# chenhaoxing/DiffUTE

Measured on AMD Instinct MI355X. Metric: 512x512 50-step denoise images/sec, higher is better.
Workload: dtype bf16; 1 GPU; SD2-inpaint UNet 50-step DDIM denoise loop, 512x512 px, batch 4 per GPU, glyph context [B,577,1024], ctx K/V cached per image (BASELINE configs[1]); VAE encode/decode not in the timed region; global_batch=4, denoise_steps=50, parallelism=replicas x1 (no collective), weights=random-init SD2-inpainting shapes (865,925,124 params), bf16 packed

## Files before the change

### diffute_amd/csrc/exec.h

```cpp
#pragma once
#include <map>
#include <string>
#include <unordered_map>
#include <vector>
#include "kernels.h"

struct PackRule {
  enum Kind { COPY_F32, CONV, LINEAR, GEGLU_W, GEGLU_B } kind = COPY_F32;
  size_t dst = 0;
  int rows = 0, cols = 0;
  int ks = 0, ld = 0, koff = 0;
};
struct ParamEntry { std::string name; int shape[4]; PackRule rule; };

class ParamTable {
 public:
  size_t reserve(size_t bytes) { size_t o = total_; total_ += align_up(bytes, 256); return o; }
  void add(const std::string& name, std::initializer_list<int> shape, const PackRule& r) {
    ParamEntry e; e.name = name; int i = 0; for (int k = 0; k < 4; ++k) e.shape[k] = 0;
    for (int s : shape) e.shape[i++] = s;
    e.rule = r; index_[name] = (int)entries_.size(); entries_.push_back(e);
  }
  size_t f32(const std::string& name, int n) {
    PackRule r; r.kind = PackRule::COPY_F32; r.dst = reserve((size_t)n * 4); r.rows = n; add(name, {n}, r); return r.dst;
// ... 85 lines not shown

struct ConvOpts {
  int ksize = 3, stride = 1, pad = 1, ups = 0;
  const float* bias2 = nullptr;
  int ldw = 0;
  int ups2 = 0;
  const float* bias = nullptr;
  const float* rowbias = nullptr; int ldrb = 0;
  const Tn* res = nullptr;
  const Tn* sc0 = nullptr; const Tn* sc1 = nullptr;
  int out_f32 = 0;
  int stats = 0;
  int defer = 0;
};

class Exec {
 public:
  hipStream_t stream = nullptr;
  bool dry = false;
  int rc = 0;
  Workspace ws;
  bool f32 = false;
  bool ff_fold = dmx_ff_fold_enabled();
  const char* masters = nullptr;
  struct Weights {
    const char* base; size_t mul;
    template <typename T> const T* at(size_t off) const { return (const T*)(base + off * mul); }
  };
  Weights weights(const char* arena) const { return f32 ? Weights{masters, 2} : Weights{arena, 1}; }
  static Exec dry_run(bool f32 = false) { Exec e; e.dry = true; e.f32 = f32; e.ws.reset(nullptr, 0, true); return e; }
  static Exec on(hipStream_t stream, void* ws, size_t bytes, bool f32 = false) { Exec e; e.stream = stream; e.f32 = f32; e.ws.reset(ws, bytes, false); return e; }
  TapSink* taps = nullptr;
  size_t esz() const { return f32 ? 4 : 2; }
  bf16* col(const Tn& t, int c) const { return (bf16*)((char*)t.p + (size_t)c * esz()); }
  void tap(const Tn& t);

  Tn make(int B, int H, int W, int C) {
    Tn t; t.B = B; t.H = H; t.W = W; t.C = C; t.ld = C;
    t.p = (bf16*)ws.alloc((size_t)B * H * W * C * esz());
    if (ws.failed() && !rc) { dmx_set_error("workspace too small"); rc = DMX_ERR_WORKSPACE; }
    return t;
  }
  void* raw(size_t bytes) {
    void* p = ws.alloc(bytes);
    if (ws.failed() && !rc) { dmx_set_error("workspace too small"); rc = DMX_ERR_WORKSPACE; }
    return p;
// ... 54 lines not shown
```

### diffute_amd/csrc/exec.hip

```cpp
#include <stdarg.h>
#include <stdio.h>
#include <string.h>
#include "exec.h"
#include <vector>

static thread_local char g_err[512] = "";
void dmx_set_error(const char* fmt, ...) {
  va_list ap; va_start(ap, fmt); vsnprintf(g_err, sizeof(g_err), fmt, ap); va_end(ap);
}
const char* dmx_get_error() { return g_err; }
static int* g_dev_err = nullptr;
int* dmx_dev_err_words() {
  static bool tried = false;
  if (!tried) {
    tried = true;
    void* p = nullptr;
    if (hipHostMalloc(&p, 64, hipHostMallocMapped | hipHostMallocCoherent) == hipSuccess && p) { memset(p, 0, 64); g_dev_err = (int*)p; }
    else (void)hipGetLastError();
  }
  return g_dev_err;
}
int dmx_poll_device_error() {
  volatile int* e = g_dev_err;
  if (!e || !e[0]) return DMX_OK;
// ... 10 lines not shown
  else if (k == DMX_DEVK_ATTN_PEER)
    dmx_set_error("device error: attention (balanced schedule) slot %d gave up after 40 ms waiting for the partial (O, m, l) record of slot %d for query block %d (%d slots) - "
                  "the slots in front of it did not run; the result of that launch is invalid", blk, d0, d1, d2);
  else
    dmx_set_error("device error %d raised by block %d (%d, %d, %d)", k, blk, d0, d1, d2);
  e[0] = 0;
  for (int i = 2; i < 8; ++i) e[i] = 0;
  __atomic_thread_fence(__ATOMIC_SEQ_CST);
  e[1] = 0;
  return DMX_ERR_DEVICE;
}
extern "C" int dmx_device_error(void) { return dmx_poll_device_error(); }
int dmx_check_launch(const char* what) {
  hipError_t e = hipGetLastError();
  if (e != hipSuccess) { dmx_set_error("launch of %s failed: %s", what, hipGetErrorString(e)); return DMX_ERR_HIP; }
  const int rc = dmx_poll_device_error();
  if (rc) {
    char first[400]; strncpy(first, dmx_get_error(), sizeof(first) - 1); first[sizeof(first) - 1] = 0;
    dmx_set_error("%s [surfaced at the launch check of %s, which itself was enqueued correctly; the walk it belongs to is abandoned]", first, what ? what : "?");
  }
  return rc;
}

static int g_plan_sw[DMX_SW_COUNT] = {1, 1, 1, 1, 1, 1, 1, 0, 1, 1, 1, 1};
void dmx_plan_switch(int slot, int value) { if (slot >= 0 && slot < DMX_SW_COUNT) g_plan_sw[slot] = value; }
void dmx_plan_epoch_bump() { ++g_plan_sw[DMX_SW_OVERRIDES]; }
extern "C" int dmx_plan_epoch(void) {
  unsigned h = 2166136261u;
  for (int i = 0; i < DMX_SW_COUNT; ++i) h = (h ^ (unsigned)g_plan_sw[i]) * 16777619u;
  return (int)(h & 0x7fffffffu);
}

namespace {
struct ProfRec { hipEvent_t a, b; int cls; double flops, bytes; char tag[96]; char sym[112]; };
struct ProfSym { char sym[112]; int cls; double n, ms, flops, bytes; };
std::vector<ProfSym> g_prof_syms;
bool g_prof_on = false;
std::vector<ProfRec> g_prof;
char g_prof_path[512] = "";
}
ProfScope::ProfScope(ProfClass c, hipStream_t s, double flops, double bytes, const char* tag) {
  if (!g_prof_on) return;
  ProfRec r; r.cls = c; r.flops = flops; r.bytes = bytes; r.tag[0] = 0; r.sym[0] = 0;
  if (tag) { strncpy(r.tag, tag, sizeof(r.tag) - 1); r.tag[sizeof(r.tag) - 1] = 0; }
  if (hipEventCreate(&r.a) != hipSuccess || hipEventCreate(&r.b) != hipSuccess) return;
  (void)hipEventRecord(r.a, s);
  slot = (int)g_prof.size(); g_prof.push_back(r);
// ... 98 lines not shown
  auto nxt = free_.lower_bound(o);
  if (nxt != free_.end() && o + sz == nxt->first) { sz += nxt->second; nxt = free_.erase(nxt); }
  if (nxt != free_.begin()) {
    auto prv = std::prev(nxt);
    if (prv->first + prv->second == o) { o = prv->first; sz += prv->second; free_.erase(prv); }
  }
  free_[o] = sz;
}

static int g_gn_producer_stats = 1;
extern "C" int dmx_set_gn_producer_stats(int on) { const int old = g_gn_producer_stats; g_gn_producer_stats = on; dmx_plan_switch(DMX_SW_GN_STATS, on); return old; }

static int g_defer_reduce = 1;
extern "C" int dmx_set_defer_reduce(int on) { const int old = g_defer_reduce; g_defer_reduce = on; dmx_plan_switch(DMX_SW_DEFER, on); return old; }

static int g_halo_conv = 1;
extern "C" int dmx_set_halo_conv(int on) { const int old = g_halo_conv; g_halo_conv = on; dmx_plan_switch(DMX_SW_HALO, on); return old; }
bool dmx_halo_conv_enabled() { return g_halo_conv != 0; }

static int g_ff_fold = 1;
extern "C" int dmx_set_ff_fold(int on) { const int old = g_ff_fold; g_ff_fold = on ? 1 : 0; dmx_plan_switch(DMX_SW_FF_FOLD, g_ff_fold); return old; }
bool dmx_ff_fold_enabled() { return g_ff_fold != 0; }

#ifdef DMX_PROBES
static int g_pool_memset_nodes = 0;
static unsigned long long* g_pool_counts = nullptr;
extern "C" int dmx_set_pool_memset_nodes(int mode) { const int old = g_pool_memset_nodes; g_pool_memset_nodes = mode; return old; }
__global__ __launch_bounds__(256) void dmx_probe_count_nonzero_kernel(const u32x4* p, size_t n16, unsigned long long* dst) {
  unsigned long long c = 0;
  for (size_t i = (size_t)blockIdx.x * blockDim.x + threadIdx.x; i < n16; i += (size_t)gridDim.x * blockDim.x) { const u32x4 v = p[i]; c += (v.x | v.y | v.z | v.w) != 0u; }
  if (c) atomicAdd(dst, c);
  if (blockIdx.x == 0 && threadIdx.x == 0 && p[n16 - 1].x != 0u) { dst[4] = p[n16 - 1].x | ((unsigned long long)p[n16 - 1].y << 32); dst[5] = p[n16 / 2].x | ((unsigned long long)p[n16 / 2].y << 32); }
}
extern "C" int dmx_probe_pool_counts(unsigned long long* host8, int reset) {
  if (!g_pool_counts) { DMX_HIP(hipMalloc(&g_pool_counts, 128)); DMX_HIP(hipMemset(g_pool_counts, 0, 128)); }
  DMX_HIP(hipDeviceSynchronize());
  if (host8) DMX_HIP(hipMemcpy(host8, g_pool_counts, 64, hipMemcpyDeviceToHost));
  if (reset) DMX_HIP(hipMemset(g_pool_counts, 0, 128));
  return DMX_OK;
}
#endif
bool Exec::zero_pool(void* p, size_t bytes, int which) {
  if (dry || rc) return !rc;
#ifdef DMX_PROBES
  if (g_pool_memset_nodes & 1) {
    const bool count = (g_pool_memset_nodes & 2) && g_pool_counts;
// ... 93 lines not shown
  Tn y = make(x0.B, x0.H, x0.W, C);
  if (f32) {
    if (!dry && !rc)
      rc = dmx_groupnorm_f32_launch((const float*)x0.p, x0.ld, x0.C, x1 ? (const float*)x1->p : nullptr, x1 ? x1->ld : 0, C, groups, x0.B, x0.H * x0.W,
                                    gamma, beta, eps, silu ? 1 : 0, (float*)y.p, y.ld, stream);
    return y;
  }
  if (x1) flush(*x1);
  if (x0.cst && (!x1 || x1->cst)) {
    flush(x0);
    if (!dry && !rc) {
      GroupNormArgs a{};
      a.x0 = x0.p; a.ldx0 = x0.ld; a.c0 = x0.C;
      a.x1 = x1 ? x1->p : nullptr; a.ldx1 = x1 ? x1->ld : 0;
      a.C = C; a.groups = groups; a.B = x0.B; a.HW = x0.H * x0.W;
      a.gamma = gamma; a.beta = beta; a.eps = eps; a.silu = silu ? 1 : 0;
      a.y = y.p; a.ldy = y.ld; a.st0 = x0.cst; a.st1 = x1 ? x1->cst : x0.cst;
      char tag[96]; snprintf(tag, sizeof(tag), "rows=%d C=%d sums", x0.rows(), C);
      ProfScope ps(PROF_GNORM, stream, 0.0, 4.0 * (double)x0.rows() * C, tag);
      rc = dmx_groupnorm_sums_launch(a, stream);
    }
    return y;
  }
  const size_t pb = dmx_gn_workspace_bytes(x0.B, x0.H * x0.W, groups);
  void* part = raw(pb);
  PendRed* P = (x0.pend >= 0 && x0.pend < (int)pend_.size() && !pend_[x0.pend].done) ? &pend_[x0.pend] : nullptr;
  GroupNormArgs a{};
  a.x0 = x0.p; a.ldx0 = x0.ld; a.c0 = x0.C;
  a.x1 = x1 ? x1->p : nullptr; a.ldx1 = x1 ? x1->ld : 0;
  a.C = C; a.groups = groups; a.B = x0.B; a.HW = x0.H * x0.W;
  a.gamma = gamma; a.beta = beta; a.eps = eps; a.silu = silu ? 1 : 0;
  a.y = y.p; a.ldy = y.ld; a.partial = (float*)part;
  if (P) {
    a.red_partial = P->a.partial ? P->a.partial : (const float*)8;
    a.red_splitk = P->a.splitk; a.red_mn = (long long)P->a.M * P->a.N;
    a.red_bias = P->a.bias; a.red_rowbias = P->a.rowbias; a.red_ldrb = P->a.ldrb; a.red_rpg = P->a.rows_per_group;
    a.red_res = P->a.res; a.red_ldres = P->a.ldres;
    if (P->a.N != x0.C || P->a.ldo != x0.ld || !dmx_gn_red_ok(a)) {
      flush(x0); P = nullptr;
      a.red_partial = nullptr; a.red_splitk = 0;
    }
  }
  if (!dry && !rc) {
    const bool one = dmx_gn_single_launch(a);
    char tag[96]; snprintf(tag, sizeof(tag), "rows=%d C=%d%s%s", x0.rows(), C, one ? " slab" : "", P ? " + split-K reduce" : "");
    ProfScope ps(PROF_GNORM, stream, 0.0, (one ? 4.0 : 6.0) * (double)x0.rows() * C, tag);
    if (!rc) rc = dmx_groupnorm_launch(a, stream);
  }
  if (P) { if (P->wsp) ws.release(P->wsp); P->wsp = nullptr; P->done = true; }
  ws.release(part);
  return y;
}

Tn Exec::conv(const Tn& x0, const Tn* x1, const bf16* w, int Cout, const ConvOpts& o, void* f32_out) {
  flush(x0); if (x1) flush(*x1); if (o.sc0) flush(*o.sc0); if (o.sc1) flush(*o.sc1); if (o.res) flush(*o.res);
  int OH = x0.H, OW = x0.W;
  if (o.ups) { OH *= 2; OW *= 2; }
  if (o.stride > 1) { OH /= o.stride; OW /= o.stride; }
  Tn y; y.B = x0.B; y.H = OH; y.W = OW; y.C = Cout; y.ld = Cout;
  if (!o.out_f32) y = make(x0.B, OH, OW, Cout);
  if (f32) {
    GemmF32Args a{};
    a.x0 = (const float*)x0.p; a.ldx0 = x0.ld; a.cx0 = x0.C;
    a.x1 = x1 ? (const float*)x1->p : (const float*)x0.p; a.ldx1 = x1 ? x1->ld : x0.ld;
    a.Cin = x0.C + (x1 ? x1->C : 0);
    a.ksize = o.ksize; a.stride = o.stride; a.pad = o.pad; a.ups = o.ups;
    a.direct = (o.ksize == 1 && o.stride == 1 && !o.ups) ? 1 : 0;
    a.IH = x0.H; a.IW = x0.W; a.OH = OH; a.OW = OW;
    a.Ktaps = o.ksize * o.ksize * a.Cin; a.K = a.Ktaps;
    if (o.sc0) {
      a.s0 = (const float*)o.sc0->p; a.lds0 = o.sc0->ld; a.cs0 = o.sc0->C;
      a.s1 = o.sc1 ? (const float*)o.sc1->p : a.s0; a.lds1 = o.sc1 ? o.sc1->ld : o.sc0->ld;
      a.K += o.sc0->C + (o.sc1 ? o.sc1->C : 0);
// ... 11 lines not shown
  a.x1 = x1 ? x1->p : x0.p; a.ldx1 = x1 ? x1->ld : x0.ld;
  a.Cin = x0.C + (x1 ? x1->C : 0);
  a.ksize = o.ksize; a.stride = o.stride; a.pad = o.pad; a.ups = o.ups;
  a.direct = (o.ksize == 1 && o.stride == 1 && !o.ups) ? 1 : 0;
  a.IH = x0.H; a.IW = x0.W; a.OH = OH; a.OW = OW;
  a.Ktaps = o.ksize * o.ksize * a.Cin;
  a.K = a.Ktaps;
  if (o.sc0) {
    a.s0 = o.sc0->p; a.lds0 = o.sc0->ld; a.cs0 = o.sc0->C;
    a.s1 = o.sc1 ? o.sc1->p : o.sc0->p; a.lds1 = o.sc1 ? o.sc1->ld : o.sc0->ld;
    a.K += o.sc0->C + (o.sc1 ? o.sc1->C : 0);
  }
  a.w = w; a.ldw = a.K;
  a.M = x0.B * OH * OW; a.N = Cout;
  if (o.ups && o.ups2) {
    a.ups = 0; a.ups2 = 1; a.ksize = 2; a.pad = 0;
    a.OH = x0.H; a.OW = x0.W; a.M4 = x0.rows();
    a.Ktaps = a.K = 4 * a.Cin; a.ldw = a.K; a.w_phase_stride = (long long)Cout * a.K;
  }
  a.bias = o.bias; a.rowbias = o.rowbias; a.rows_per_group = OH * OW; a.ldrb = o.ldrb;
  if (o.res) { a.res = o.res->p; a.ldres = o.res->ld; }
  a.out = o.out_f32 ? f32_out : (void*)y.p; a.ldo = Cout; a.out_f32 = o.out_f32;
  if (o.stats && !o.out_f32) want_stats(a, y, (o.ups && o.ups2) ? x0.H * x0.W : OH * OW, x0.B);
  run_gemm(a, (o.defer && g_defer_reduce && !(o.defer == 2 && g_defer_reduce == 2) && !o.out_f32 && !a.ups2) ? &y : nullptr);
  return y;
}

bool dmx_halo_conv_enabled();
void Exec::ensure_stats(Tn& t) {
  if (rc || f32 || t.cst || !dmx_halo_conv_enabled() || !g_gn_producer_stats || (t.C & 7) || (t.ld & 7)) return;
  if (!dmx_conv_halo_wants_stats(t.H, t.W, g_halo_conv != 1)) return;
  flush(t);
  long long* st = stat_slice(t.B, t.C);
  if (!st) return;
  if (!dry && !rc) rc = dmx_colstats_launch(t.p, t.ld, t.B, t.H * t.W, t.C, st, stream);
  t.cst = st;
}

Tn Exec::conv_gn(const Tn& x0, const Tn* x1, const float* gamma, const float* beta, int groups, float eps, const bf16* w, int Cout, const ConvOpts& o) {
  HaloConvArgs a{};
  bool fused = !f32 && dmx_halo_conv_enabled() && o.ksize == 3 && o.stride == 1 && o.pad == 1 && !o.ups && !o.out_f32 && x0.cst && (!x1 || x1->cst);
  if (fused) {
    a.x0 = x0.p; a.ldx0 = x0.ld; a.cx0 = x0.C; a.Cin = x0.C + (x1 ? x1->C : 0);
    if (x1) { a.x1 = x1->p; a.ldx1 = x1->ld; }
    a.B = x0.B; a.H = x0.H; a.W = x0.W;
    a.gn = 1; a.silu = 1; a.groups = groups; a.eps = eps; a.st0 = x0.cst; a.st1 = x1 ? x1->cst : nullptr; a.gamma = gamma; a.beta = beta;
    if (o.sc0) {
// ... 274 lines not shown
```

### diffute_amd/csrc/kernels.h

```cpp
#pragma once
#include <vector>
#include "common.h"
#include "../../include/diffute_hip.h"

enum ProfClass { PROF_GEMM128 = 0, PROF_GEMM64 = 1, PROF_SPLITK = 2, PROF_ATTN = 3, PROF_GNORM = 4, PROF_LNORM = 5,
                 PROF_OTHER = 6, PROF_GEMM256 = 7, PROF_WGRAD = 8, PROF_GEMM256WS = 9,
                 PROF_GEMM_CFG0 = 10 , PROF_XFCHAIN = 26 , PROF_HALO = 27 , PROF_SKINNY = 28 , PROF_NCLASS = 29 };
int n_cus();
enum DmxPlanSwitch { DMX_SW_EXCLUSIVE = 0, DMX_SW_GN_STATS, DMX_SW_DEFER, DMX_SW_HALO, DMX_SW_PREFETCH, DMX_SW_XF_CHAIN, DMX_SW_HALO_WS, DMX_SW_OVERRIDES, DMX_SW_SKINNY, DMX_SW_HALO_PEERS, DMX_SW_ATTN_BALANCED, DMX_SW_FF_FOLD, DMX_SW_COUNT };
void dmx_plan_switch(int slot, int value);
void dmx_plan_epoch_bump();
int dmx_exclusive_device();
void dmx_profile_note_symbol(const char* sym);
struct ProfScope {
  ProfScope(ProfClass c, hipStream_t s, double flops, double bytes, const char* tag = nullptr);
  ~ProfScope();
  int slot = -1;
  hipStream_t stream_ = nullptr;
};

struct GemmArgs {
  const bf16* x0; const bf16* x1;
  int ldx0, ldx1;
  int cx0;
  int direct;
  int IH, IW, OH, OW;
  int stride, pad, ups, ksize;
  int ups2, M4; long long w_phase_stride;
  int Cin;
  int Ktaps;
  const bf16* s0; const bf16* s1; int lds0, lds1, cs0;
  const bf16* w; int ldw;
// ... 12 lines not shown
  int ln_C; float ln_eps;
  long long* timing;
  int dbg;
  const void* pf[2]; int pf_bytes[2]; int pf_dump_off;
  float* partial; int splitk, kt_per_split;
  int defer_reduce;
  int persist; int* flags; int* err;
  long long* colstats; int cs_rows;
  const bf16* zeros;
};
int dmx_gemm_launch(GemmArgs a, void* workspace, size_t workspace_bytes, hipStream_t stream);
size_t dmx_gemm_workspace_bytes(const GemmArgs& a);
void dmx_gemm_plan(const GemmArgs& a, int* tn, int* splitk, int* ktps);
int dmx_zero_page(const bf16** out);
void dmx_gemm_plan_override_set(int M, int N, int K, int st, int ups, int cfg, int sk);
bool dmx_gemm_colstats_ok(const GemmArgs& a);
int dmx_gemm_persist_blocks(const GemmArgs& a);
int dmx_gemm_tiles_n(const GemmArgs& a);
int dmx_ups_phase_weights_launch(const bf16* w3, int ldw3, bf16* wp, int N, int Cin, hipStream_t stream);
int dmx_ln_fold_launch(const bf16* w_raw, bf16* w_out, const float* gamma, const float* beta, const float* bias,
                       float* c1, float* c2, int N, int K, hipStream_t stream);
int dmx_compose_linear_launch(const bf16* wpo, const bf16* wf2, const float* bf2, const float* bpo, bf16* w_out, float* b_out, int C, int K, hipStream_t stream);
bool dmx_ff_fold_enabled();

struct HaloConvArgs {
  const bf16* x0; const bf16* x1; int ldx0, ldx1;
  int cx0, Cin;
  int B, H, W;
  int gn, silu, groups; float eps;
  const long long* st0; const long long* st1;
  const float* gamma; const float* beta;
  const bf16* s0; const bf16* s1; int lds0, lds1, cs0, Csc;
  const bf16* w; int ldw;
  int N;
  const float* bias; const float* rowbias; int ldrb;
  const bf16* res; int ldres;
  bf16* out; int ldo;
  long long* colstats;
  int force_split;
  int force_bn;
  int force_waves;
  int dbg; long long* timing;
  const void* pf[2]; int pf_bytes[2];
  int TH, TW, splits, xcd_tile_major; float* slabs; int* flags; const bf16* zeros; int* err;
  int peers_local;
  int tiles_x, tiles_img, tiles_m, ncombo, cpg;
// ... 60 lines not shown
  float* out; int ldout;
  int accumulate;
  int splits, rows_per_split;
  const bf16* zeros;
};
size_t dmx_wgrad_workspace_bytes(const WgradArgs& a);
int dmx_wgrad_launch(WgradArgs a, void* workspace, size_t workspace_bytes, hipStream_t stream);
size_t dmx_colsum_ws_bytes(int groups, int rows_per_group, int N);
int dmx_colsum_launch(const bf16* dy, int lddy, int groups, int rows_per_group, int N, float* out, int ldo, int accumulate,
                      void* workspace, size_t workspace_bytes, hipStream_t stream);

struct GroupNormArgs {
  const bf16* x0; const bf16* x1; int ldx0, ldx1; int c0;
  int C, groups; int B, HW;
  const float* gamma; const float* beta; float eps; int silu;
  bf16* y; int ldy;
  float* partial;
  float* stats_out;
  float* coef;
  const long long* st0; const long long* st1;
  int nchunk, rows_per_chunk;
  const float* red_partial; int red_splitk; long long red_mn; const float* red_bias; const float* red_rowbias; int red_ldrb, red_rpg;
  const bf16* red_res; int red_ldres;
};
bool dmx_gn_red_ok(GroupNormArgs a);
size_t dmx_gn_workspace_bytes(int B, int HW, int groups);
int dmx_groupnorm_launch(GroupNormArgs a, hipStream_t stream);
int dmx_groupnorm_sums_launch(GroupNormArgs a, hipStream_t stream);
bool dmx_gn_single_launch(GroupNormArgs a);
int dmx_splitk_reduce_launch(const GemmArgs& a, hipStream_t stream);
int dmx_layernorm_launch(const bf16* x, int ldx, bf16* y, int ldy, const float* gamma, const float* beta,
                         int rows, int C, float eps, hipStream_t stream);

struct GroupNormBwdArgs {
  const bf16* x0; const bf16* x1; int ldx0, ldx1; int c0;
  int C, groups; int B, HW;
  const float* gamma; const float* beta; int silu;
  const float* stats;
  const bf16* dy; int lddy;
  bf16* dx0; int lddx0; bf16* dx1; int lddx1;
  const bf16* res0; int ldres0; const bf16* res1; int ldres1;
  float* dgamma; float* dbeta; int accumulate;
  float* part;
  float* ab; int nchunk, rows_per_chunk;
};
size_t dmx_gn_bwd_workspace_bytes(int B, int HW, int C);
// ... 158 lines not shown
```

### diffute_amd/csrc/norm.hip

```cpp
#include "common.h"
#include "kernels.h"
#include <stdlib.h>

__device__ __forceinline__ const bf16* gn_src(const GroupNormArgs& p, size_t row, int c) {
  return (c < p.c0) ? (p.x0 + row * p.ldx0 + c) : (p.x1 + row * p.ldx1 + (c - p.c0));
}

__global__ __launch_bounds__(1024) void dmx_gn_stats_kernel(const GroupNormArgs p) {
  extern __shared__ float sm[];
  const int oc = p.C >> 3;
  const int R = blockDim.x / oc;
  const int t = threadIdx.x;
  const int r = t / oc, co = t - r * oc;
  const int b = blockIdx.y, chunk = blockIdx.x;
  const int row0 = chunk * p.rows_per_chunk;
  const int row1 = min(row0 + p.rows_per_chunk, p.HW);
  float s[8], ss[8];
#pragma unroll
  for (int i = 0; i < 8; ++i) { s[i] = 0.f; ss[i] = 0.f; }
  const size_t base = (size_t)b * p.HW;
  int row = row0 + r;
  for (; row + 3 * R < row1; row += 4 * R) {
    u32x4 v[4];
#pragma unroll
// ... 156 lines not shown
  __shared__ float AF[2][128];
  const int t = threadIdx.x, nw = (blockDim.x + 63) >> 6;
  const int G = p.groups;
  int b, g;
  if ((G & 7) == 0) { const int gpx = G >> 3, j = blockIdx.x >> 3; b = j / gpx; g = (blockIdx.x & 7) * gpx + j % gpx; }
  else { b = blockIdx.x / G; g = blockIdx.x - b * G; }
  const int cpg = p.C / G;
  const int within = t % SU, r = t / SU;
  const bool active = r < R;
  const int c = g * cpg + within * 2 * VEC;
  const bf16* src; int ld;
  if (c < p.c0) { src = p.x0 + c; ld = p.ldx0; } else { src = p.x1 + (c - p.c0); ld = p.ldx1; }
  src += (size_t)b * p.HW * ld;
  V v[NU];
  float s = 0.f;
  const char* const safe = (const char*)src;
  const char* lp = (const char*)(src + (size_t)r * ld);
  const size_t lstep = (size_t)R * ld * 2;
  bool red_done = false;
  if constexpr (RED) {
    if (p.red_partial && c < p.c0) {
      red_done = true;
      constexpr int NE = 2 * VEC;
#pragma unroll
      for (int k = 0; k < NU; ++k) {
        const int pr = r + k * R;
        const bool ok = active && pr < p.HW;
        V o;
#pragma unroll
        for (int i = 0; i < VEC; ++i) gn_set<VEC>(o, i, 0u);
        if (ok) {
          const size_t m = (size_t)b * p.HW + pr;
          const float* q = p.red_partial + m * (size_t)p.c0 + c;
          float bvv[NE], rbv[NE]; unsigned int rw[VEC];
#pragma unroll
          for (int e = 0; e < NE; e += 2) {
            const f32x2 t2 = p.red_bias ? *(const f32x2*)(p.red_bias + c + e) : (f32x2){0.f, 0.f};
            const f32x2 t3 = p.red_rowbias ? *(const f32x2*)(p.red_rowbias + (size_t)(m / p.red_rpg) * p.red_ldrb + c + e) : (f32x2){0.f, 0.f};
            bvv[e] = t2.x; bvv[e + 1] = t2.y; rbv[e] = t3.x; rbv[e + 1] = t3.y;
          }
#pragma unroll
          for (int i = 0; i < VEC; ++i) rw[i] = p.red_res ? *(const unsigned int*)(p.red_res + m * (size_t)p.red_ldres + c + 2 * i) : 0u;
          float a[NE];
#pragma unroll
          for (int e = 0; e < NE; e += 2) { const f32x2 t2 = *(const f32x2*)(q + e); a[e] = t2.x; a[e + 1] = t2.y; }
          int j = 1;
// ... 4 lines not shown
#pragma unroll
              for (int e = 0; e < NE / 2; ++e) tt[u][e] = *(const f32x2*)(q + (size_t)(j + u) * (size_t)p.red_mn + 2 * e);
#pragma unroll
            for (int u = 0; u < 4; ++u)
#pragma unroll
              for (int e = 0; e < NE / 2; ++e) { a[2 * e] += tt[u][e].x; a[2 * e + 1] += tt[u][e].y; }
          }
          for (; j < p.red_splitk; ++j) {
            const float* qj = q + (size_t)j * (size_t)p.red_mn;
#pragma unroll
            for (int e = 0; e < NE; e += 2) { const f32x2 t2 = *(const f32x2*)(qj + e); a[e] += t2.x; a[e + 1] += t2.y; }
          }
#pragma unroll
          for (int e = 0; e < NE; ++e) a[e] = a[e] + bvv[e] + rbv[e];
          if (p.red_res) {
#pragma unroll
            for (int i = 0; i < VEC; ++i) { a[2 * i] += h2f_lo(rw[i]); a[2 * i + 1] += h2f_hi(rw[i]); }
          }
#pragma unroll
          for (int i = 0; i < VEC; ++i) gn_set<VEC>(o, i, pack_bf2(a[2 * i], a[2 * i + 1]));
          *(GV*)(p.x0 + m * (size_t)p.ldx0 + c) = o;
        }
        v[k] = o;
      }
    }
  }
  if (!red_done) {
#pragma unroll
  for (int k = 0; k < NU; ++k) {
    const bool ok = active && (r + k * R < p.HW);
    asm volatile("" : "+v"(lp));
    v[k] = *(const GV*)((ok && !(dbg & 2)) ? lp : safe);
    lp += lstep;
    __builtin_amdgcn_sched_barrier(0);
  }
  }
#pragma unroll
  for (int k = 0; k < NU; ++k) {
    const bool ok = active && (r + k * R < p.HW);
    float u = 0.f;
#pragma unroll
    for (int i = 0; i < VEC; ++i) {
      const unsigned int w = gn_dw<VEC>(v[k], i);
      u += h2f_lo(w) + h2f_hi(w);
    }
    s += ok ? u : 0.f;
// ... 90 lines not shown
  GN_SLAB(2, 2) GN_SLAB(2, 4) GN_SLAB(2, 8) GN_SLAB(2, 16)
  GN_SLAB(4, 1) GN_SLAB(4, 2) GN_SLAB(4, 4) GN_SLAB(4, 8)
#undef GN_SLAB
  return false;
}

static bool gn_two_pass_forced() {
#ifdef DMX_PROBES
  static const bool off = getenv("DMX_GN_TWO_PASS") != nullptr;
  return off;
#else
  return false;
#endif
}
bool dmx_gn_single_launch(GroupNormArgs a) {
  if (a.c0 >= a.C || a.x1 == nullptr) { a.c0 = a.C; a.x1 = a.x0; a.ldx1 = a.ldx0; }
  return !gn_two_pass_forced() && a.C % a.groups == 0 && gn_slab_launch(a, nullptr, true);
}

bool dmx_gn_red_ok(GroupNormArgs a) {
  if (!a.red_partial || a.red_splitk < 2 || a.C % a.groups) return false;
  if (a.c0 >= a.C || a.x1 == nullptr) { a.c0 = a.C; a.x1 = a.x0; a.ldx1 = a.ldx0; }
  const int cpg = a.C / a.groups;
  if (a.c0 % cpg || a.c0 % 8 || a.red_rpg <= 0) return false;
  return !gn_two_pass_forced() && gn_slab_launch(a, nullptr, true);
}

#define GN_MAX_CHUNKS 256
size_t dmx_gn_workspace_bytes(int B, int HW, int groups) {
  (void)HW;
  return (size_t)B * GN_MAX_CHUNKS * groups * 2 * sizeof(float) + (size_t)B * 2560 * 2 * sizeof(float);
}

int dmx_groupnorm_sums_launch(GroupNormArgs a, hipStream_t stream) {
  DMX_REQUIRE(a.C % 8 == 0 && a.C % a.groups == 0 && a.C <= 2560 && a.groups <= 64, "groupnorm: C=%d / groups=%d unsupported", a.C, a.groups);
  DMX_REQUIRE(a.c0 % 8 == 0 && a.ldx0 % 8 == 0 && a.ldy % 8 == 0, "groupnorm: strides/splits must be multiples of 8");
  if (a.c0 >= a.C || a.x1 == nullptr) { a.c0 = a.C; a.x1 = a.x0; a.ldx1 = a.ldx0; a.st1 = a.st0; }
  DMX_REQUIRE(a.st0 != nullptr && a.st1 != nullptr, "groupnorm: producer statistics missing");
  const int oc = a.C / 8;
  int R = 1024 / oc; if (R > 16) R = 16; if (R < 1) R = 1;
  const int threads = oc * R;
  int rpb = 8 * R;
  while (rpb > R && (long)cdiv(a.HW, rpb) * a.B < 512) rpb -= R;
  a.partial = nullptr; a.nchunk = 0;
  hipLaunchKernelGGL(dmx_gn_apply_kernel, dim3(cdiv(a.HW, rpb), a.B), dim3(threads), (size_t)2 * a.C * sizeof(double), stream, a, rpb);
  return dmx_check_launch("dmx_gn_apply_kernel");
}
// ... 133 lines not shown
```

### diffute_amd/csrc/unet.hip

```cpp
#include <stdlib.h>
#include <math.h>
#include "unet_model.h"

namespace {

void build_resnet(dmx_unet* u, ResW& r, const std::string& p, int cin, int cout, bool temb) {
  resnet_build(u->pt, r, p, cin, cout);
  if (temb) { r.temb_off = u->tproj_total; u->tproj_total += cout; }
}

void build_xf(dmx_unet* u, XfW& x, const std::string& p, int C, int heads) {
  ParamTable& pt = u->pt;
  const int ctx = u->cfg.cross_attention_dim;
  x.C = C; x.heads = heads;
  x.ng = pt.f32(p + "norm.weight", C); x.nb = pt.f32(p + "norm.bias", C);
  x.wpi = pt.linear(p + "proj_in.weight", C, C); x.bpi = pt.f32(p + "proj_in.bias", C);
  const std::string t = p + "transformer_blocks.0.";
  x.l1g = pt.f32(t + "norm1.weight", C); x.l1b = pt.f32(t + "norm1.bias", C);
  x.wqkv_raw = pt.reserve((size_t)3 * C * C * 2);
  pt.linear_at(t + "attn1.to_q.weight", C, C, x.wqkv_raw, C);
  pt.linear_at(t + "attn1.to_k.weight", C, C, x.wqkv_raw + (size_t)C * C * 2, C);
  pt.linear_at(t + "attn1.to_v.weight", C, C, x.wqkv_raw + (size_t)2 * C * C * 2, C);
  x.wqkv = pt.reserve((size_t)3 * C * C * 2);
  x.c1_qkv = pt.reserve((size_t)3 * C * 4); x.c2_qkv = pt.reserve((size_t)3 * C * 4);
// ... 470 lines not shown
  Tn held;
  auto xf = [&](const XfW& w, Tn& y) {
    Tn z = f.xformer(w, y);
    if (z.pend >= 0) held = y; else ex.drop(y);
    y = z;
  };
  auto drop_held = [&]() { if (held.p) { ex.drop(held); held = Tn(); } };
  for (int i = 0; i < (shallow ? 1 : 4); ++i) {
    for (int j = 0; j < L; ++j) {
#ifdef DMX_PROBES
      static const bool fine = getenv("DMX_TAPS_FINE") != nullptr;
#else
      constexpr bool fine = false;
#endif
      Tn y = f.resnet(u->down_res[i][j], h, nullptr);
      drop_held();
      if (fine) ex.tap(y);
      if (cfg.down_has_attn[i]) { xf(u->down_xf[i][j], y); if (fine) ex.tap(y); }
      ex.ensure_stats(y);
      h = y; skips.push_back(h);
    }
    if (i < 3 && !shallow) {
      ConvOpts o; o.stride = 2; o.pad = 1; o.bias = f.W<float>(u->down_ds[i].b); o.stats = 1;
      h = ex.conv(h, nullptr, f.W<bf16>(u->down_ds[i].w), boc[i], o);
      drop_held();
      ex.ensure_stats(h);
      skips.push_back(h);
    }
    ex.tap(h);
  }
  if (shallow) drop_held();
  Tn mid_in;
  if (!shallow) {
    Tn z = f.resnet(u->mid_res[0], h, nullptr);
    drop_held();
    xf(u->mid_xf, z);
    ex.ensure_stats(z);
    h = f.resnet(u->mid_res[1], z, nullptr); mid_in = z;
    drop_held();
    ex.tap(h);
  } else {
    h = Tn(); h.p = sc_t; h.B = B; h.H = H; h.W = W; h.C = boc[1]; h.ld = boc[1];
    h.cst = sc.has_stats ? (ex.dry ? (const long long*)8 : sc_st) : nullptr;
  }
  for (int i = shallow ? 3 : 0; i < 4; ++i) {
    for (int j = 0; j < L + 1; ++j) {
      Tn s = skips.back(); skips.pop_back();
      Tn y = f.resnet(u->up_res[i][j], h, &s);
      drop_held();
      if (i == 0 && j == 0) ex.drop(mid_in);
      if (!(shallow && j == 0)) ex.drop(h);
      ex.drop(s);
      if (cfg.up_has_attn[i]) xf(u->up_xf[i][j], y);
      ex.ensure_stats(y);
      h = y;
    }
    if (i < 3) {
      const bool direct = ex.f32;
      ConvOpts o; o.ups = 1; o.ups2 = direct ? 0 : 1; o.bias = f.W<float>(u->up_us[i].b); o.stats = 1;
      Tn y = ex.conv(h, nullptr, direct ? f.W<bf16>(u->up_us[i].w) : u->at<bf16>(u->up_us[i].wp), boc[3 - i], o);
      drop_held();
      ex.ensure_stats(y);
      ex.drop(h); h = y;
      if (i == 2 && sc.mode == DMX_STEP_CACHE_FILL) {
        ex.flush(h);
        sc.has_stats = h.cst != nullptr;
        if (!ex.dry && !ex.rc) {
          const size_t nt = step_cache_tensor_bytes(u, B, H, W) / 16, ns = sc.has_stats ? step_cache_stat_bytes(u, B) / 16 : 0;
          ProfScope ps(PROF_OTHER, ex.stream, 0.0, 32.0 * (double)(nt + ns), "step cache store");
          const size_t blocks = (nt + ns + 255) / 256;
          hipLaunchKernelGGL(dmx_step_cache_store_kernel, dim3((unsigned)(blocks < 2048 ? blocks : 2048)), dim3(256), 0, ex.stream,
                             (const u32x4*)h.p, (u32x4*)sc_t, nt, (const u32x4*)h.cst, (u32x4*)sc_st, ns);
          ex.rc = dmx_check_launch("dmx_step_cache_store_kernel");
        }
      }
    }
    ex.tap(h);
  }
  Tn t = ex.groupnorm(h, nullptr, f.W<float>(u->cno_g), f.W<float>(u->cno_b), cfg.norm_num_groups, 1e-5f, true);
  drop_held();
  ex.drop(h);
  float* eps_nhwc = (float*)ex.raw((size_t)B * H * W * cfg.out_channels * 4);
// ... 40 lines not shown
  if (it != u->step_cache_stats.end()) return it->second;
  Exec ex = Exec::dry_run();
  StepCache sc; sc.mode = DMX_STEP_CACHE_FILL;
  unet_run(u, ex, dry_call(c.t_count, c.ctx_len, c.B, c.H, c.W), sc);
  if (u->step_cache_stats.size() > 256) u->step_cache_stats.clear();
  return u->step_cache_stats[key] = sc.has_stats;
}

int step_cache_record(dmx_unet* u, const UNetCall& c, void* cache, size_t cache_bytes, int mode, const char* who, StepCache* sc) {
  DMX_REQUIRE(mode == DMX_STEP_CACHE_FILL || mode == DMX_STEP_CACHE_USE, "%s: unknown step cache mode %d", who, mode);
  DMX_REQUIRE(cache != nullptr, "%s: null step cache", who);
  DMX_REQUIRE(((size_t)cache & 15) == 0, "%s: the step cache must be 16-byte aligned", who);
  DMX_REQUIRE(cache_bytes >= dmx_unet_step_cache_bytes(u, c.B, c.H, c.W), "%s: step cache too small (%zu bytes, needs %zu)", who, cache_bytes,
              dmx_unet_step_cache_bytes(u, c.B, c.H, c.W));
  sc->mode = mode; sc->buf = cache;
  sc->has_stats = mode == DMX_STEP_CACHE_USE && step_cache_has_stats(u, c);
  return DMX_OK;
}

}

static size_t walk_peak(dmx_unet* u, const UNetCall& c, const StepCache& sc) {
  size_t need = 0;
  for (int k = 0; k < 2; ++k) {
    Exec ex = Exec::dry_run();
    if (k) ex.ff_fold = !ex.ff_fold;
    StepCache s = sc;
    unet_run(u, ex, c, s);
    if (ex.ws.peak() > need) need = ex.ws.peak();
  }
  return need;
}

extern "C" size_t dmx_unet_workspace_bytes(dmx_unet* u, int B, int H, int W, int ctx_len) {
  if (!u) return 0;
  size_t need = walk_peak(u, dry_call(1, ctx_len, B, H, W), StepCache());
  Exec e2 = Exec::dry_run();
  project_context(u, e2, nullptr, 0, 0, B, B, ctx_len, nullptr);
  if (e2.ws.peak() > need) need = e2.ws.peak();
  return need + 4096;
}

extern "C" int dmx_unet_forward(dmx_unet* u, UNET_CALL_PARAMS, void* workspace, size_t workspace_bytes, dmx_stream_t stream) {
  const UNetCall c = UNET_CALL_RECORD;
  if (const int rc = unet_check_call(u, c, workspace, "unet_forward")) return rc;
  return forward_eager(u, c, StepCache(), workspace, workspace_bytes, (hipStream_t)stream);
}

extern "C" int dmx_unet_forward_taps(dmx_unet* u, UNET_CALL_PARAMS, void* workspace, size_t workspace_bytes,
// ... 92 lines not shown
```

### include/diffute_hip.h

```cpp
#ifndef DIFFUTE_HIP_H
#define DIFFUTE_HIP_H

#include <stddef.h>
#include <stdint.h>

#ifdef __cplusplus
extern "C" {
#endif

#define DMX_OK 0
#define DMX_ERR_ARG (-1)
#define DMX_ERR_HIP (-2)
#define DMX_ERR_UNSUPPORTED (-3)
#define DMX_ERR_WORKSPACE (-4)

typedef void* dmx_stream_t;
typedef struct dmx_unet dmx_unet;
typedef struct dmx_vae dmx_vae;

int dmx_version(void);
const char* dmx_last_error(void);
int dmx_device_error(void);
int dmx_test_raise_device_error(int code, dmx_stream_t stream);
int dmx_test_occupy_cus(int blocks, long long ticks, dmx_stream_t stream);
// ... 2 lines not shown
int dmx_test_transpose_bf16(const void* in, int ldin, void* out, int ldout, int R, int C, dmx_stream_t stream);
typedef struct dmx_test_tr_job { const void* in; int ldin; void* out; int ldout; int R, C; } dmx_test_tr_job;
int dmx_test_transpose_batch(const dmx_test_tr_job* h_jobs, int njobs, void* table, size_t table_bytes, dmx_stream_t stream);
int dmx_test_add_bf16(const void* a, int lda, const void* b, int ldb, void* out, int ldo, int rows, int C, dmx_stream_t stream);
int dmx_test_softmax_rows(const float* s, int lds, void* p, int ldp, int rows, int n, float scale, dmx_stream_t stream);
int dmx_test_softmax_bwd_rows(const void* p, int ldp, const float* dp, int lddp, void* ds, int ldds, int rows, int n, float scale, dmx_stream_t stream);
int dmx_test_pointwise_small_fwd(const void* x, int ldx, const void* w, int ldw, const float* bias, void* y, int ldy, int M, int Cin, int Cout,
                                 int out_f32, dmx_stream_t stream);
size_t dmx_test_pointwise_small_bwd_workspace_bytes(int M, int Cin, int Cout);
int dmx_test_pointwise_small_bwd(const void* x, int ldx, const float* dy, int lddy, const void* w, int ldw, void* dx, int lddx,
                                 float* dw, int lddw, float* db, int M, int Cin, int Cout, void* workspace, size_t workspace_bytes, dmx_stream_t stream);
int dmx_test_linear_small_bwd(const float* x, int ldx, const float* dy, int lddy, const void* w, int ldw, float* dw, int lddw, float* db, int db_stride,
                              float* dx, int lddx, int B, int N, int K, int silu_in, int accumulate, dmx_stream_t stream);
int dmx_test_slice_cast(const float* in, int ldin, void* out, int ldo, int M, int C, dmx_stream_t stream);
int dmx_test_mode_bwd(const void* dz, int lddz, float* dmom, int M, int C, dmx_stream_t stream);
int dmx_test_bf16_to_f32_rows(const void* in, int ldin, float* out, int M, int C, dmx_stream_t stream);
int dmx_test_ln_fold(const void* w_raw, void* w_out, const float* gamma, const float* beta, const float* bias, float* c1, float* c2,
                     int N, int K, dmx_stream_t stream);
int dmx_test_cast_pad_rows(const void* in, int in_is_16, void* out, int B, int S, int Spad, int C, dmx_stream_t stream);
int dmx_test_compose_linear(const void* wpo, const void* wf2, const float* bf2, const float* bpo, void* w_out, float* b_out, int C, int K, dmx_stream_t stream);
size_t dmx_test_folded_tail_gn_workspace_bytes(int B, int HW, int C, int groups, int mode);
int dmx_test_folded_tail_gn(const void* g, const void* h3, const void* x, const void* wfpo, const float* bfpo, const float* gamma, const float* beta,
                            int B, int HW, int C, int groups, int mode, void* y_out, void* t_out, void* workspace, size_t workspace_bytes, dmx_stream_t stream);


typedef struct dmx_gemm_desc {
  const void* x0; const void* x1;
  int ldx0, ldx1, cx0;
  int direct;
  int IH, IW, OH, OW;
  int stride, pad, ups, ksize;
  int Cin;
  int Ktaps;
  const void* s0; const void* s1;
  int lds0, lds1, cs0;
  const void* w; int ldw;
  int M, N, K;
  const float* bias;
  const float* rowbias;
  int rows_per_group, ldrb;
  const void* res; int ldres;
  void* out; int ldo; int out_f32;
  int geglu;
  int force_tn, force_splitk;
  int group_m;
  long long* timing;
// ... 91 lines not shown

typedef struct {
  int M, C;
  const void* x; int ldx;
  const void* res; int ldres;
  const void* w0; const float* b0;
  void* h_out; int ldh;
  const void* w1;
  const float* c1; const float* c2;
  void* y; int ldy;
  const void* wf1;
  const void* wf2; const float* bf2;
  const void* wpo; const float* bpo;
  const void* xres; int ldxres;
  float eps;
  int dbg; long long* timing;
  long long* colstats; int cs_rows;
  const long long* gn_st; const float* gn_gamma; const float* gn_beta; int gn_groups; int gn_rows; float gn_eps;
} dmx_xf_chain_desc;
int dmx_xf_chain_ok(int M, int C);
int dmx_xf_chain(const dmx_xf_chain_desc* d, int mode, dmx_stream_t stream);
int dmx_set_xf_chain(int on);
int dmx_set_ff_fold(int on);
int dmx_set_weight_prefetch(int on);

int dmx_groupnorm_train(const void* x0, int ldx0, const void* x1, int ldx1, int c0, int C, int groups,
                        int B, int HW, const float* gamma, const float* beta, float eps, int silu,
                        void* y, int ldy, float* stats, void* workspace, size_t workspace_bytes, dmx_stream_t stream);
size_t dmx_groupnorm_bwd_workspace_bytes(int B, int HW, int C);
int dmx_groupnorm_bwd(const void* x0, int ldx0, const void* x1, int ldx1, int c0, int C, int groups, int B, int HW,
                      const float* gamma, const float* beta, int silu, const float* stats,
                      const void* dy, int lddy, void* dx0, int lddx0, void* dx1, int lddx1,
                      const void* res0, int ldres0, const void* res1, int ldres1,
                      float* dgamma, float* dbeta, int accumulate,
                      void* workspace, size_t workspace_bytes, dmx_stream_t stream);
size_t dmx_layernorm_bwd_workspace_bytes(int rows, int C);
int dmx_layernorm_bwd(const void* x, int ldx, const void* dy, int lddy, const float* gamma, void* dx, int lddx,
                      const void* res, int ldres, float* dgamma, float* dbeta, int accumulate,
                      int rows, int C, float eps, void* workspace, size_t workspace_bytes, dmx_stream_t stream);
int dmx_geglu_fwd(const void* h, int ldh, void* y, int ldy, int rows, int C2, dmx_stream_t stream);
int dmx_geglu_bwd(const void* h, int ldh, const void* dy, int lddy, void* dh, int lddh, int rows, int C2, dmx_stream_t stream);

int dmx_layernorm(const void* x, int ldx, void* y, int ldy, const float* gamma, const float* beta,
                  int rows, int C, float eps, dmx_stream_t stream);

int dmx_attention_fwd(const void* q, int ldq, const void* k, int ldk, int kv_rows,
// ... 460 lines not shown
```

Baseline: 12.20 images/s.

## Hand off split-K conv reductions for downsample/upsample convs into the following GroupNorm

Adds a default-on gn_handoff switch that lets the stride-2 downsample convs and the first upsample conv defer their split-K reduction into the consumer GroupNorm kernel. GroupNorm can now accept reductions whose channel split straddles a group boundary, and gains a dedicated NU==1 reduce path that prefetches several split-K partials at once. The GN partial-stats workspace is skipped when the reduction is fused. This removes a separate reduce pass and a round trip through memory, at the cost of more complex GN kernels and a larger dry-run peak search.

```diff
diff --git a/diffute_amd/csrc/exec.h b/diffute_amd/csrc/exec.h
--- a/diffute_amd/csrc/exec.h
+++ b/diffute_amd/csrc/exec.h
@@ -131,6 +131,7 @@
   Workspace ws;
   bool f32 = false;
   bool ff_fold = dmx_ff_fold_enabled();
+  bool gn_handoff = dmx_gn_handoff_enabled();
   const char* masters = nullptr;
   struct Weights {
     const char* base; size_t mul;
diff --git a/diffute_amd/csrc/exec.hip b/diffute_amd/csrc/exec.hip
--- a/diffute_amd/csrc/exec.hip
+++ b/diffute_amd/csrc/exec.hip
@@ -56,7 +56,7 @@
   return rc;
 }
 
-static int g_plan_sw[DMX_SW_COUNT] = {1, 1, 1, 1, 1, 1, 1, 0, 1, 1, 1, 1};
+static int g_plan_sw[DMX_SW_COUNT] = {1, 1, 1, 1, 1, 1, 1, 0, 1, 1, 1, 1, 1};
 void dmx_plan_switch(int slot, int value) { if (slot >= 0 && slot < DMX_SW_COUNT) g_plan_sw[slot] = value; }
 void dmx_plan_epoch_bump() { ++g_plan_sw[DMX_SW_OVERRIDES]; }
 extern "C" int dmx_plan_epoch(void) {
@@ -201,6 +201,10 @@
 extern "C" int dmx_set_ff_fold(int on) { const int old = g_ff_fold; g_ff_fold = on ? 1 : 0; dmx_plan_switch(DMX_SW_FF_FOLD, g_ff_fold); return old; }
 bool dmx_ff_fold_enabled() { return g_ff_fold != 0; }
 
+static int g_gn_handoff = 1;
+extern "C" int dmx_set_gn_handoff(int on) { const int old = g_gn_handoff; g_gn_handoff = on ? 1 : 0; dmx_plan_switch(DMX_SW_GN_HANDOFF, g_gn_handoff); return old; }
+bool dmx_gn_handoff_enabled() { return g_gn_handoff != 0; }
+
 #ifdef DMX_PROBES
 static int g_pool_memset_nodes = 0;
 static unsigned long long* g_pool_counts = nullptr;
@@ -340,25 +344,26 @@
     }
     return y;
   }
-  const size_t pb = dmx_gn_workspace_bytes(x0.B, x0.H * x0.W, groups);
-  void* part = raw(pb);
+  void* part = gn_handoff ? nullptr : raw(dmx_gn_workspace_bytes(x0.B, x0.H * x0.W, groups));
   PendRed* P = (x0.pend >= 0 && x0.pend < (int)pend_.size() && !pend_[x0.pend].done) ? &pend_[x0.pend] : nullptr;
   GroupNormArgs a{};
   a.x0 = x0.p; a.ldx0 = x0.ld; a.c0 = x0.C;
   a.x1 = x1 ? x1->p : nullptr; a.ldx1 = x1 ? x1->ld : 0;
   a.C = C; a.groups = groups; a.B = x0.B; a.HW = x0.H * x0.W;
   a.gamma = gamma; a.beta = beta; a.eps = eps; a.silu = silu ? 1 : 0;
-  a.y = y.p; a.ldy = y.ld; a.partial = (float*)part;
+  a.y = y.p; a.ldy = y.ld;
   if (P) {
     a.red_partial = P->a.partial ? P->a.partial : (const float*)8;
     a.red_splitk = P->a.splitk; a.red_mn = (long long)P->a.M * P->a.N;
     a.red_bias = P->a.bias; a.red_rowbias = P->a.rowbias; a.red_ldrb = P->a.ldrb; a.red_rpg = P->a.rows_per_group;
-    a.red_res = P->a.res; a.red_ldres = P->a.ldres;
+    a.red_res = P->a.res; a.red_ldres = P->a.ldres; a.red_straddle = gn_handoff ? 1 : 0;
     if (P->a.N != x0.C || P->a.ldo != x0.ld || !dmx_gn_red_ok(a)) {
       flush(x0); P = nullptr;
       a.red_partial = nullptr; a.red_splitk = 0;
     }
   }
+  if (gn_handoff && !P) part = raw(dmx_gn_workspace_bytes(x0.B, x0.H * x0.W, groups));
+  a.partial = part ? (float*)part : (float*)8;
   if (!dry && !rc) {
     const bool one = dmx_gn_single_launch(a);
     char tag[96]; snprintf(tag, sizeof(tag), "rows=%d C=%d%s%s", x0.rows(), C, one ? " slab" : "", P ? " + split-K reduce" : "");
@@ -366,7 +371,7 @@
     if (!rc) rc = dmx_groupnorm_launch(a, stream);
   }
   if (P) { if (P->wsp) ws.release(P->wsp); P->wsp = nullptr; P->done = true; }
-  ws.release(part);
+  if (part) ws.release(part);
   return y;
 }
 
@@ -424,7 +429,7 @@
   if (o.res) { a.res = o.res->p; a.ldres = o.res->ld; }
   a.out = o.out_f32 ? f32_out : (void*)y.p; a.ldo = Cout; a.out_f32 = o.out_f32;
   if (o.stats && !o.out_f32) want_stats(a, y, (o.ups && o.ups2) ? x0.H * x0.W : OH * OW, x0.B);
-  run_gemm(a, (o.defer && g_defer_reduce && !(o.defer == 2 && g_defer_reduce == 2) && !o.out_f32 && !a.ups2) ? &y : nullptr);
+  run_gemm(a, (o.defer && g_defer_reduce && !(o.defer == 2 && g_defer_reduce == 2) && !o.out_f32) ? &y : nullptr);
   return y;
 }
 
diff --git a/diffute_amd/csrc/kernels.h b/diffute_amd/csrc/kernels.h
--- a/diffute_amd/csrc/kernels.h
+++ b/diffute_amd/csrc/kernels.h
@@ -7,7 +7,7 @@
                  PROF_OTHER = 6, PROF_GEMM256 = 7, PROF_WGRAD = 8, PROF_GEMM256WS = 9,
                  PROF_GEMM_CFG0 = 10 , PROF_XFCHAIN = 26 , PROF_HALO = 27 , PROF_SKINNY = 28 , PROF_NCLASS = 29 };
 int n_cus();
-enum DmxPlanSwitch { DMX_SW_EXCLUSIVE = 0, DMX_SW_GN_STATS, DMX_SW_DEFER, DMX_SW_HALO, DMX_SW_PREFETCH, DMX_SW_XF_CHAIN, DMX_SW_HALO_WS, DMX_SW_OVERRIDES, DMX_SW_SKINNY, DMX_SW_HALO_PEERS, DMX_SW_ATTN_BALANCED, DMX_SW_FF_FOLD, DMX_SW_COUNT };
+enum DmxPlanSwitch { DMX_SW_EXCLUSIVE = 0, DMX_SW_GN_STATS, DMX_SW_DEFER, DMX_SW_HALO, DMX_SW_PREFETCH, DMX_SW_XF_CHAIN, DMX_SW_HALO_WS, DMX_SW_OVERRIDES, DMX_SW_SKINNY, DMX_SW_HALO_PEERS, DMX_SW_ATTN_BALANCED, DMX_SW_FF_FOLD, DMX_SW_GN_HANDOFF, DMX_SW_COUNT };
 void dmx_plan_switch(int slot, int value);
 void dmx_plan_epoch_bump();
 int dmx_exclusive_device();
@@ -66,6 +66,7 @@
                        float* c1, float* c2, int N, int K, hipStream_t stream);
 int dmx_compose_linear_launch(const bf16* wpo, const bf16* wf2, const float* bf2, const float* bpo, bf16* w_out, float* b_out, int C, int K, hipStream_t stream);
 bool dmx_ff_fold_enabled();
+bool dmx_gn_handoff_enabled();
 
 struct HaloConvArgs {
   const bf16* x0; const bf16* x1; int ldx0, ldx1;
@@ -172,6 +173,7 @@
   int nchunk, rows_per_chunk;
   const float* red_partial; int red_splitk; long long red_mn; const float* red_bias; const float* red_rowbias; int red_ldrb, red_rpg;
   const bf16* red_res; int red_ldres;
+  int red_straddle;
 };
 bool dmx_gn_red_ok(GroupNormArgs a);
 size_t dmx_gn_workspace_bytes(int B, int HW, int groups);
diff --git a/diffute_amd/csrc/norm.hip b/diffute_amd/csrc/norm.hip
--- a/diffute_amd/csrc/norm.hip
+++ b/diffute_amd/csrc/norm.hip
@@ -202,6 +202,52 @@
     if (p.red_partial && c < p.c0) {
       red_done = true;
       constexpr int NE = 2 * VEC;
+      if constexpr (NU == 1) {
+        constexpr int PB = 3;
+        const int sk = p.red_splitk;
+        const bool ok = active && r < p.HW;
+        const size_t m = (size_t)b * p.HW + (ok ? r : 0);
+        const float* q = p.red_partial + m * (size_t)p.c0 + c;
+        const float* bp = p.red_bias ? p.red_bias + c : q;
+        const float* rp = p.red_rowbias ? p.red_rowbias + (size_t)((unsigned)m / (unsigned)p.red_rpg) * p.red_ldrb + c : q;
+        const unsigned int* sp = p.red_res ? (const unsigned int*)(p.red_res + m * (size_t)p.red_ldres + c) : (const unsigned int*)q;
+        float a[NE], bvv[NE], rbv[NE]; unsigned int rw[VEC];
+#pragma unroll
+        for (int e = 0; e < NE; e += 2) {
+          const f32x2 t2 = *(const f32x2*)(bp + e), t3 = *(const f32x2*)(rp + e);
+          bvv[e] = p.red_bias ? t2.x : 0.f; bvv[e + 1] = p.red_bias ? t2.y : 0.f; rbv[e] = p.red_rowbias ? t3.x : 0.f; rbv[e + 1] = p.red_rowbias ? t3.y : 0.f;
+        }
+#pragma unroll
+        for (int i = 0; i < VEC; ++i) rw[i] = sp[i];
+        for (int j = 0; j < sk; j += PB) {
+          f32x2 tt[PB][NE / 2];
+#pragma unroll
+          for (int u = 0; u < PB; ++u) {
+            const float* qu = q + (size_t)(j + u < sk ? j + u : sk - 1) * (size_t)p.red_mn;
+#pragma unroll
+            for (int e = 0; e < NE / 2; ++e) tt[u][e] = *(const f32x2*)(qu + 2 * e);
+          }
+#pragma unroll
+          for (int u = 0; u < PB; ++u) {
+            const bool first = j + u == 0, add = j + u < sk;
+#pragma unroll
+            for (int e = 0; e < NE / 2; ++e) {
+              a[2 * e] = first ? tt[u][e].x : add ? a[2 * e] + tt[u][e].x : a[2 * e];
+              a[2 * e + 1] = first ? tt[u][e].y : add ? a[2 * e + 1] + tt[u][e].y : a[2 * e + 1];
+            }
+          }
+        }
+#pragma unroll
+        for (int e = 0; e < NE; ++e) a[e] = a[e] + bvv[e] + rbv[e];
+        V o;
+#pragma unroll
+        for (int i = 0; i < VEC; ++i) {
+          const float r0 = p.red_res ? a[2 * i] + h2f_lo(rw[i]) : a[2 * i], r1 = p.red_res ? a[2 * i + 1] + h2f_hi(rw[i]) : a[2 * i + 1];
+          gn_set<VEC>(o, i, ok ? pack_bf2(r0, r1) : 0u);
+        }
+        if (ok) *(GV*)(p.x0 + m * (size_t)p.ldx0 + c) = o;
+        v[0] = o;
+      } else {
 #pragma unroll
       for (int k = 0; k < NU; ++k) {
         const int pr = r + k * R;
@@ -252,6 +298,7 @@
           *(GV*)(p.x0 + m * (size_t)p.ldx0 + c) = o;
         }
         v[k] = o;
+      }
       }
     }
   }
@@ -388,7 +435,7 @@
   if (!a.red_partial || a.red_splitk < 2 || a.C % a.groups) return false;
   if (a.c0 >= a.C || a.x1 == nullptr) { a.c0 = a.C; a.x1 = a.x0; a.ldx1 = a.ldx0; }
   const int cpg = a.C / a.groups;
-  if (a.c0 % cpg || a.c0 % 8 || a.red_rpg <= 0) return false;
+  if ((!a.red_straddle && a.c0 % cpg) || a.c0 % 8 || a.red_rpg <= 0) return false;
   return !gn_two_pass_forced() && gn_slab_launch(a, nullptr, true);
 }
 
diff --git a/diffute_amd/csrc/unet.hip b/diffute_amd/csrc/unet.hip
--- a/diffute_amd/csrc/unet.hip
+++ b/diffute_amd/csrc/unet.hip
@@ -516,6 +516,7 @@
     }
     if (i < 3 && !shallow) {
       ConvOpts o; o.stride = 2; o.pad = 1; o.bias = f.W<float>(u->down_ds[i].b); o.stats = 1;
+      o.defer = ex.gn_handoff ? 2 : 0;
       h = ex.conv(h, nullptr, f.W<bf16>(u->down_ds[i].w), boc[i], o);
       drop_held();
       ex.ensure_stats(h);
@@ -552,6 +553,7 @@
     if (i < 3) {
       const bool direct = ex.f32;
       ConvOpts o; o.ups = 1; o.ups2 = direct ? 0 : 1; o.bias = f.W<float>(u->up_us[i].b); o.stats = 1;
+      o.defer = (ex.gn_handoff && i == 0) ? 2 : 0;
       Tn y = ex.conv(h, nullptr, direct ? f.W<bf16>(u->up_us[i].w) : u->at<bf16>(u->up_us[i].wp), boc[3 - i], o);
       drop_held();
       ex.ensure_stats(y);
@@ -638,9 +640,10 @@
 
 static size_t walk_peak(dmx_unet* u, const UNetCall& c, const StepCache& sc) {
   size_t need = 0;
-  for (int k = 0; k < 2; ++k) {
+  for (int k = 0; k < 4; ++k) {
     Exec ex = Exec::dry_run();
-    if (k) ex.ff_fold = !ex.ff_fold;
+    if (k & 1) ex.ff_fold = !ex.ff_fold;
+    if (k & 2) ex.gn_handoff = !ex.gn_handoff;
     StepCache s = sc;
     unet_run(u, ex, c, s);
     if (ex.ws.peak() > need) need = ex.ws.peak();
diff --git a/include/diffute_hip.h b/include/diffute_hip.h
--- a/include/diffute_hip.h
+++ b/include/diffute_hip.h
@@ -48,6 +48,10 @@
 size_t dmx_test_folded_tail_gn_workspace_bytes(int B, int HW, int C, int groups, int mode);
 int dmx_test_folded_tail_gn(const void* g, const void* h3, const void* x, const void* wfpo, const float* bfpo, const float* gamma, const float* beta,
                             int B, int HW, int C, int groups, int mode, void* y_out, void* t_out, void* workspace, size_t workspace_bytes, dmx_stream_t stream);
+size_t dmx_test_conv_gn_handoff_workspace_bytes(int kind, int B, int H, int W, int Cin, int Cout, int C1, int groups);
+int dmx_test_conv_gn_handoff(int kind, int handoff, const void* x, const void* w, const float* bias, const void* res, const void* x1, int C1,
+                             const float* gamma, const float* beta, int B, int H, int W, int Cin, int Cout, int groups,
+                             void* y_out, void* t_out, void* workspace, size_t workspace_bytes, dmx_stream_t stream);
 
 
 typedef struct dmx_gemm_desc {
@@ -185,6 +189,7 @@
 int dmx_xf_chain(const dmx_xf_chain_desc* d, int mode, dmx_stream_t stream);
 int dmx_set_xf_chain(int on);
 int dmx_set_ff_fold(int on);
+int dmx_set_gn_handoff(int on);
 int dmx_set_weight_prefetch(int on);
 
 int dmx_groupnorm_train(const void* x0, int ldx0, const void* x1, int ldx1, int c0, int C, int groups,
```

Result: no change. 12.22 images/s (median of 4 runs) (+0.2%).
